# markomih/SplatFields

Hardware: AMD Instinct MI355X
Metric: splats*px rasterized/sec (fwd+bwd) (higher is better)
Workload: dtype f32

## Files before the change

splatfields_amd/csrc/api.hip:

```cpp
#include <cstdint>
#include <cstdio>
#include <cstdlib>
#include <cstring>
#include <atomic>
#include <chrono>
#include <thread>
#include <mutex>
#include <string>
#include <vector>
#include "host_api.h"
#include "kernels.h"

namespace {

thread_local std::string g_last_error;
thread_local long long g_last_longest = -1;

struct ProfRec { int stage; hipEvent_t a, b; bool ended; unsigned long long serial; };
unsigned long long g_prof_serial = 0;
bool g_prof_on = false;
std::vector<ProfRec> g_prof;
std::mutex g_prof_mutex;
const char* kStageNames[SR_PROFILE_STAGES] = {"preprocess", "scan", "emit", "sort_tiles", "render_forward",
                                              "render_backward", "preprocess_backward"};

}

namespace sr {

int fail(const std::string& msg) { g_last_error = msg; return 1; }

int check_hip(hipError_t e, const char* what) {
    if (e == hipSuccess) return 0;
    return fail(std::string(what) + ": " + hipGetErrorString(e));
}

StageTimer::StageTimer(int stage, hipStream_t s) : st(s) {
    if (!g_prof_on) return;
    ProfRec r; r.stage = stage; r.ended = false;
    if (hipEventCreate(&r.a) != hipSuccess || hipEventCreate(&r.b) != hipSuccess) return;
    hipEventRecord(r.a, st);
    std::lock_guard<std::mutex> lock(g_prof_mutex);
    serial = ++g_prof_serial;
    r.serial = serial;
    g_prof.push_back(r); idx = 0;
    end = r.b;
}
StageTimer::~StageTimer() {
    if (idx < 0) return;
    std::lock_guard<std::mutex> lock(g_prof_mutex);
    for (auto& r : g_prof)
        if (r.serial == serial) { hipEventRecord(end, st); r.ended = true; break; }
}

}

using sr::fail; using sr::check_hip; using sr::StageTimer;

namespace {

struct StatusBlock { uint32_t* pinned = nullptr; uint32_t* pinned_dev = nullptr; uint32_t seq = 0; hipStream_t stream = nullptr; int dev = 0; };
thread_local StatusBlock g_sync[64];
std::mutex g_ticket_mutex;
std::vector<StatusBlock*> g_ticket_free[64];
std::atomic<long long> g_counters[4];

int status_block_init(StatusBlock& b, int dev) {
    if (hipHostMalloc(reinterpret_cast<void**>(&b.pinned), 64, hipHostMallocCoherent) != hipSuccess &&
        hipHostMalloc(reinterpret_cast<void**>(&b.pinned), 64, hipHostMallocDefault) != hipSuccess) return fail("hipHostMalloc failed");
    void* dp = nullptr;
    if (hipHostGetDevicePointer(&dp, b.pinned, 0) != hipSuccess) { hipHostFree(b.pinned); b.pinned = nullptr; return fail("hipHostGetDevicePointer failed"); }
    b.pinned_dev = static_cast<uint32_t*>(dp);
    for (int i = 0; i < 16; ++i) b.pinned[i] = 0u;
    b.dev = dev; b.seq = 0;
    return 0;
}
uint32_t status_block_arm(StatusBlock& b, hipStream_t st) {
    b.seq = b.seq + 1u == 0u ? 1u : b.seq + 1u;
    b.stream = st;
    return b.seq;
}
int status_block_wait(StatusBlock& b, bool* waited) {
    volatile uint32_t* p = b.pinned;
    auto ready = [&] { return p[2] == b.seq && p[3] == b.seq; };
    if (waited) *waited = false;
    if (!ready()) {
        if (waited) *waited = true;
        const auto t0 = std::chrono::steady_clock::now();
        for (unsigned spins = 0; !ready(); ++spins) {
            if (spins > 4096u) std::this_thread::yield();
            if ((spins & 0xfffu) == 0xfffu && std::chrono::steady_clock::now() - t0 > std::chrono::seconds(2)) {
                SR_TRY(check_hip(hipStreamSynchronize(b.stream), "wait for the instance count"));
                if (!ready()) return fail("the instance count of the forward never reached the host (k_scan_small did not run?)");
            }
        }
    }
    std::atomic_thread_fence(std::memory_order_acquire);
    return 0;
}

int current_device(int* dev) {
    if (hipGetDevice(dev) != hipSuccess || *dev < 0 || *dev >= 64) return fail("hipGetDevice failed");
    return 0;
}

int thread_block(StatusBlock** out) {
    int dev = 0;
    SR_TRY(current_device(&dev));
    *out = &g_sync[dev];
    return (*out)->pinned ? 0 : status_block_init(**out, dev);
}

int ticket_acquire(StatusBlock** out) {
    int dev = 0;
    SR_TRY(current_device(&dev));
    {
        std::lock_guard<std::mutex> lock(g_ticket_mutex);
        if (!g_ticket_free[dev].empty()) { *out = g_ticket_free[dev].back(); g_ticket_free[dev].pop_back(); return 0; }
    }
    StatusBlock* t = new StatusBlock;
    if (int rc = status_block_init(*t, dev)) { delete t; return rc; }
    g_counters[3].fetch_add(1, std::memory_order_relaxed);
    *out = t;
    return 0;
}
void ticket_recycle(StatusBlock* t) {
    std::lock_guard<std::mutex> lock(g_ticket_mutex);
    g_ticket_free[t->dev].push_back(t);
}

std::atomic<int> g_bwd_kernel{[] {
    const char* sel = getenv("SPLATRASTER_BWD");
    return !sel ? 0 : (std::string(sel) == "wave" ? 1 : (std::string(sel) == "quads" ? 2 : 0));
}()};


struct CallContext { const SrView* view = nullptr; const SrSplats* splats = nullptr; const char* file = nullptr;
                     const float* dL_dcolor = nullptr; const float* dL_ddepth = nullptr; const float* dL_dalpha = nullptr; };
thread_local CallContext g_call;

void dump_record(FILE* f, const char* name, const void* dev, size_t bytes, bool on_device) {
    char tag[16] = {0};
    std::strncpy(tag, name, 15);
    std::vector<char> host;
    uint64_t n = 0;
    if (dev && bytes) {
        host.resize(bytes);
        if (!on_device) { std::memcpy(host.data(), dev, bytes); n = bytes; }
        else if (hipMemcpy(host.data(), dev, bytes, hipMemcpyDeviceToHost) == hipSuccess) n = bytes;
        else (void)hipGetLastError();
    }
    std::fwrite(tag, 1, 16, f); std::fwrite(&n, 8, 1, f);
    if (n) std::fwrite(host.data(), 1, (size_t)n, f);
}

void dump_snapshot(const char* stage) {
    const CallContext& c = g_call;
    if (!c.view || !c.splats || !c.file) return;
    FILE* f = std::fopen(c.file, "wb");
    if (!f) return;
    char head[8] = {'S', 'R', 'S', 'N', 'A', 'P', '1', 0}, st[32] = {0};
    std::strncpy(st, stage, 31);
    std::fwrite(head, 1, 8, f); std::fwrite(st, 1, 32, f);
    const SrView* v = c.view; const SrSplats* s = c.splats;
    const int32_t vi[4] = {v->image_height, v->image_width, v->sh_degree, v->sh_coeffs};
    const float vf[3] = {v->tanfovx, v->tanfovy, v->scale_modifier};
    char vb[32]; std::memcpy(vb, vi, 16); std::memcpy(vb + 16, vf, 12); const int32_t pf = v->prefiltered; std::memcpy(vb + 28, &pf, 4);
    dump_record(f, "view", vb, 32, false);
    const int32_t n = s->count;
    dump_record(f, "count", &n, 4, false);
    dump_record(f, "viewmatrix", v->viewmatrix, 64, true); dump_record(f, "projmatrix", v->projmatrix, 64, true);
    dump_record(f, "campos", v->campos, 12, true); dump_record(f, "bg", v->bg, 12, true);
    const size_t N = (size_t)(n > 0 ? n : 0);
    dump_record(f, "means3D", s->means3D, N * 12, true); dump_record(f, "opacities", s->opacities, N * 4, true);
    dump_record(f, "scales", s->scales, N * 12, true); dump_record(f, "rotations", s->rotations, N * 16, true);
    dump_record(f, "cov3D_precomp", s->cov3D_precomp, N * 24, true);
    dump_record(f, "shs", s->shs, s->shs ? N * 12 * (size_t)(s->shs_rest ? 1 : v->sh_coeffs) : 0, true);
    dump_record(f, "shs_rest", s->shs_rest, N * 12 * 15, true);
    dump_record(f, "colors_precomp", s->colors_precomp, N * 12, true);
    const size_t px = (size_t)v->image_height * v->image_width;
    dump_record(f, "dL_dcolor", c.dL_dcolor, px * 12, true); dump_record(f, "dL_ddepth", c.dL_ddepth, px * 4, true);
    dump_record(f, "dL_dalpha", c.dL_dalpha, px * 4, true);
    std::fclose(f);
}

int after_launch(const SrView* view, hipStream_t st, const char* what) {
    int rc = check_hip(hipGetLastError(), what);
    if (!rc && view && view->debug) rc = check_hip(hipStreamSynchronize(st), what);
    if (rc && view && view->debug) {
        const std::string keep = g_last_error;
        dump_snapshot(what);
        g_last_error = keep + (g_call.file ? std::string(" (inputs written to ") + g_call.file + ")" : std::string());
    }
    return rc;
}

int validate(const SrView* view, const SrSplats* s) {
    if (!view || !s) return fail("null view/splats");
    if (s->count < 0) return fail("negative splat count");
    if (view->image_height <= 0 || view->image_width <= 0) return fail("image size must be positive");
    if (!view->viewmatrix || !view->projmatrix || !view->campos || !view->bg) return fail("viewmatrix/projmatrix/campos/bg must be device pointers");
    if (s->count > 0) {
        if (!s->means3D || !s->opacities) return fail("means3D/opacities missing");
        const bool has_sr = s->scales && s->rotations;
        if (has_sr == (s->cov3D_precomp != nullptr)) return fail("Please provide exactly one of either scale/rotation pair or precomputed 3D covariance!");
        if ((s->shs != nullptr) == (s->colors_precomp != nullptr)) return fail("Please provide excatly one of either SHs or precomputed colors!");
        if (s->shs) {
            if (view->sh_degree < 0 || view->sh_degree > 3) return fail("sh_degree must be 0..3");
            if (view->sh_coeffs < (view->sh_degree + 1) * (view->sh_degree + 1)) return fail("shs holds fewer coefficients than sh_degree needs");
            if (s->shs_rest) {
                if (view->sh_coeffs != 16) return fail("shs_rest (dc + rest SH tensors) needs sh_coeffs == 16");
                if ((reinterpret_cast<uintptr_t>(s->shs) | reinterpret_cast<uintptr_t>(s->shs_rest)) & 15u) return fail("shs / shs_rest must be 16-byte aligned");
            }
        } else if (s->shs_rest) return fail("shs_rest without shs");
        if (s->raw_params & ~(SR_RAW_SCALES | SR_RAW_OPACITY | SR_RAW_ROTATIONS | SR_FORWARD_ONLY)) return fail("unknown bits in raw_params");
        if (s->cov3D_precomp && (s->raw_params & (SR_RAW_SCALES | SR_RAW_ROTATIONS))) return fail("raw scales/rotations with cov3D_precomp");
    }
    if ((sr::tiles_x(view->image_width) > sr::kMaxTilesPerSide) || (sr::tiles_y(view->image_height) > sr::kMaxTilesPerSide)) return fail("image too large (more than 65520 pixels a side)");
    return 0;
}

sr::ViewK make_view(const SrView* v) {
    sr::ViewK k;
    k.H = v->image_height; k.W = v->image_width;
    k.gx = sr::tiles_x(k.W); k.gy = sr::tiles_y(k.H);
    k.tanfovx = v->tanfovx; k.tanfovy = v->tanfovy;
    k.focal_x = k.W / (2.0f * v->tanfovx); k.focal_y = k.H / (2.0f * v->tanfovy);
    k.scale_modifier = v->scale_modifier;
    k.sh_degree = v->sh_degree; k.sh_coeffs = v->sh_coeffs;
    k.viewmatrix = v->viewmatrix; k.projmatrix = v->projmatrix; k.campos = v->campos; k.bg = v->bg;
    return k;
}

sr::SplatsK make_splats(const SrSplats* s) {
    sr::SplatsK k;
    k.N = s->count; k.means3D = s->means3D; k.opacities = s->opacities; k.scales = s->scales;
    k.rotations = s->rotations; k.cov3D = s->cov3D_precomp; k.shs = s->shs; k.colors = s->colors_precomp;
    k.raw = s->raw_params; k.shs_rest = s->shs_rest;
    return k;
}

long long covered_by_hint(long long hint) { return hint <= 2048 ? 2048 : hint <= 4096 ? 4096 : hint <= 8192 ? 8192 : -1; }

struct Call {
    hipStream_t st = nullptr;
    sr::ViewK v; sr::SplatsK s;
    sr::Geom g; sr::Binning b; sr::Image im;
    void carve(const void* geom, void* binning, long long capacity, const void* image) {
        sr::carve_geom(const_cast<void*>(geom), s.N, v.H, v.W, &g);
        if (binning) sr::carve_binning(binning, capacity, &b);
        if (image) sr::carve_image(const_cast<void*>(image), v.H, v.W, &im);
    }
};

int open_call(Call& c, const CallContext& ctx, void* hip_stream) {
    SR_TRY(validate(ctx.view, ctx.splats));
    g_call = ctx;
    c.st = static_cast<hipStream_t>(hip_stream);
    c.v = make_view(ctx.view);
    c.s = make_splats(ctx.splats);
    return 0;
}

bool capacity_in_range(long long r) { return r >= 0 && r < (1ll << 32); }

}

extern "C" {

int sr_version(void) { return SR_VERSION; }
const char* sr_last_error(void) { return g_last_error.c_str(); }

size_t sr_geom_bytes(int n, int h, int w) { return sr::carve_geom(nullptr, n, h, w, nullptr); }
size_t sr_binning_bytes(long long r, int, int) { return sr::carve_binning(nullptr, r, nullptr); }
size_t sr_image_bytes(int h, int w) { return sr::carve_image(nullptr, h, w, nullptr); }
size_t sr_backward_scratch_bytes(long long r) {
    const size_t n = (size_t)(r > 0 ? r : 1);
    return sr::align_up(n * sr::kSlotFloats * sizeof(float), 256);
}

}

namespace {

int launch_stage1(const SrView* view, const sr::ViewK& v, const sr::SplatsK& s, const sr::Geom& g, int* radii, uint32_t* host_out,
                  uint32_t host_seq, hipStream_t st) {
    { StageTimer t_(0, st); sr::launch_preprocess(v, s, g, radii, st); }
    SR_TRY(after_launch(view, st, "preprocess"));
    { StageTimer t_(1, st); sr::launch_count_tiles(v, s.N, g, st); sr::launch_scan_small(v, s.N, g, host_out, host_seq, st); }
    SR_TRY(after_launch(view, st, "scan"));
    return 0;
}

int launch_stage2(const SrView* view, const sr::ViewK& v, const sr::SplatsK& s, const sr::Geom& g, const sr::Binning& b,
                  const sr::Image& im, float* out_color, float* out_depth, float* out_alpha, StatusBlock* hs, long long max_len,
                  long long expected_len, hipStream_t st) {
    { StageTimer t_(2, st); sr::launch_emit(v, s.N, g, b, st); }
    SR_TRY(after_launch(view, st, "emit"));
    if (hs) {
        g_counters[0].fetch_add(1, std::memory_order_relaxed);
        SR_TRY(status_block_wait(*hs, nullptr));
        max_len = (long long)hs->pinned[1];
        if ((long long)hs->pinned[0] > (long long)b.capacity) return 0;
    }
    { StageTimer t_(3, st); sr::launch_sort_tiles(v, g, b, max_len, expected_len, st); }
    SR_TRY(after_launch(view, st, "sort_tiles"));
    { StageTimer t_(4, st); sr::launch_render_forward(v, g, b, im, out_color, out_depth, out_alpha, st); }
    SR_TRY(after_launch(view, st, "render_forward"));
    return 0;
}

}

extern "C" {

int sr_forward_prepare(const SrView* view, const SrSplats* splats, void* geom, int* radii,
                       long long* instances_out, void* hip_stream) {
    Call c;
    SR_TRY(open_call(c, CallContext{view, splats, "snapshot_fw.dump"}, hip_stream));
    if (!geom || !instances_out || (splats->count > 0 && !radii)) return fail("null geom/radii/instances_out");
    c.carve(geom, nullptr, 0, nullptr);
    StatusBlock* hs = nullptr;
    SR_TRY(thread_block(&hs));
    SR_TRY(launch_stage1(view, c.v, c.s, c.g, radii, hs->pinned_dev, status_block_arm(*hs, c.st), c.st));
    SR_TRY(check_hip(hipStreamSynchronize(c.st), "sync after prepare"));
    *instances_out = (long long)hs->pinned[0];
    return 0;
}

int sr_forward(const SrView* view, const SrSplats* splats, void* geom, int* radii, void* binning,
               long long binning_capacity, void* image, float* out_color, float* out_depth, float* out_alpha,
               long long* instances_out, void* hip_stream) {
    Call c;
    SR_TRY(open_call(c, CallContext{view, splats, "snapshot_fw.dump"}, hip_stream));
    if (!geom || !binning || !image || !out_color || !out_depth || !instances_out || (splats->count > 0 && !radii)) return fail("null buffer");
    if (!capacity_in_range(binning_capacity)) return fail("binning capacity out of range");
    c.carve(geom, binning, binning_capacity, image);
    StatusBlock* hs = nullptr;
    SR_TRY(thread_block(&hs));
    SR_TRY(launch_stage1(view, c.v, c.s, c.g, radii, hs->pinned_dev, status_block_arm(*hs, c.st), c.st));
    SR_TRY(launch_stage2(view, c.v, c.s, c.g, c.b, c.im, out_color, out_depth, out_alpha, hs, -1, -1, c.st));
    const long long total = (long long)hs->pinned[0];
    *instances_out = total;
    g_last_longest = (long long)hs->pinned[1];
    return total > binning_capacity ? SR_NEED_CAPACITY : 0;
}

int sr_forward_render(const SrView* view, const SrSplats* splats, void* geom, void* binning,
                      long long instances, void* image, float* out_color, float* out_depth,
                      float* out_alpha, void* hip_stream) {
    Call c;
    SR_TRY(open_call(c, CallContext{view, splats, "snapshot_fw.dump"}, hip_stream));
    if (!geom || !binning || !image || !out_color || !out_depth) return fail("null buffer");
    if (!capacity_in_range(instances)) return fail("instance count out of range");
    c.carve(geom, binning, instances, image);
    return launch_stage2(view, c.v, c.s, c.g, c.b, c.im, out_color, out_depth, out_alpha, nullptr, -1, -1, c.st);
}

int sr_forward_async(const SrView* view, const SrSplats* splats, void* geom, int* radii, void* binning,
                     long long binning_capacity, long long longest_list_hint, long long longest_list_expected, void* image,
                     float* out_color, float* out_depth, float* out_alpha, void** ticket_out, void* hip_stream) {
    Call c;
    SR_TRY(open_call(c, CallContext{view, splats, "snapshot_fw.dump"}, hip_stream));
    if (!geom || !binning || !image || !out_color || !out_depth || !ticket_out || (splats->count > 0 && !radii)) return fail("null buffer");
    if (!capacity_in_range(binning_capacity)) return fail("binning capacity out of range");
    if (longest_list_hint < 0) return fail("longest_list_hint must be >= 0");
    c.carve(geom, binning, binning_capacity, image);
    const long long covered = covered_by_hint(longest_list_hint);
    c.b.sorted_up_to = covered < 0 ? 0xffffffffu : (uint32_t)covered;
    StatusBlock* t = nullptr;
    SR_TRY(ticket_acquire(&t));
    int rc = launch_stage1(view, c.v, c.s, c.g, radii, t->pinned_dev, status_block_arm(*t, c.st), c.st);
    if (!rc) rc = launch_stage2(view, c.v, c.s, c.g, c.b, c.im, out_color, out_depth, out_alpha, nullptr, covered,
                                longest_list_expected >= 0 && longest_list_expected <= longest_list_hint ? longest_list_expected : -1, c.st);
    if (rc) {
        (void)hipStreamSynchronize(c.st);
        ticket_recycle(t);
        return rc;
    }
    g_counters[1].fetch_add(1, std::memory_order_relaxed);
    *ticket_out = t;
    return 0;
}

int sr_ticket_wait(void* ticket, long long* instances_out, long long* longest_list_out) {
    if (!ticket) return fail("null ticket");
    StatusBlock* t = static_cast<StatusBlock*>(ticket);
    bool waited = false;
    const int rc = status_block_wait(*t, &waited);
    if (waited) g_counters[2].fetch_add(1, std::memory_order_relaxed);
    if (rc) {
        return rc;
    }
    if (instances_out) *instances_out = (long long)t->pinned[0];
    if (longest_list_out) *longest_list_out = (long long)t->pinned[1];
    ticket_recycle(t);
    return 0;
}

long long sr_last_longest_list(void) { return g_last_longest; }

int sr_ticket_release(void* ticket) { return sr_ticket_wait(ticket, nullptr, nullptr); }

int sr_debug_counters(long long* out4, int reset) {
    if (!out4) return fail("null pointer in sr_debug_counters");
    for (int i = 0; i < 4; ++i) out4[i] = reset ? g_counters[i].exchange(0, std::memory_order_relaxed) : g_counters[i].load(std::memory_order_relaxed);
    return 0;
}

namespace {
int backward_impl(int what, const SrView* view, const SrSplats* splats, const void* geom, void* binning,
                  long long instances, long long instances_rendered, const void* image, const int* radii,
                  const float* dL_dcolor, const float* dL_ddepth, const float* dL_dalpha, void* scratch,
                  const SrGrads* grads, int first, int count, void* hip_stream) {
    Call c;
    SR_TRY(open_call(c, CallContext{view, splats, "snapshot_bw.dump", dL_dcolor, dL_ddepth, dL_dalpha}, hip_stream));
    if (!geom || !binning || !image || !scratch) return fail("null buffer");
    if ((what & 1) && !dL_dcolor) return fail("null buffer");
    if ((what & 2) && !grads) return fail("null buffer");
    if (what & 2) {
        if (splats->count > 0 && (!radii || !grads->dL_dmeans3D || !grads->dL_dmeans2D || !grads->dL_dopacity)) return fail("null gradient output");
        if (splats->count > 0 && splats->shs && !grads->dL_dshs && !grads->dL_dcolors) return fail("dL_dshs (or dL_dcolors for the colour-gradient mode) missing");
        if (splats->count > 0 && splats->shs_rest && grads->dL_dshs && !grads->dL_dshs_rest) return fail("dL_dshs_rest missing");
        if (splats->count > 0 && splats->colors_precomp && !grads->dL_dcolors) return fail("dL_dcolors missing");
        if (splats->count > 0 && splats->cov3D_precomp && !grads->dL_dcov3D) return fail("dL_dcov3D missing");
        if (splats->count > 0 && !splats->cov3D_precomp && (!grads->dL_dscales || !grads->dL_drotations)) return fail("dL_dscales/dL_drotations missing");
        if (first < 0 || count < 0 || (first % sr::kBlock) != 0) return fail("splat range must start at a multiple of 256");
    }
    if (splats->raw_params & SR_FORWARD_ONLY) return fail("the forward of these buffers was run with SR_FORWARD_ONLY");
    c.carve(geom, binning, instances, image);
    const hipStream_t st = c.st;
    const sr::SplatsK& s = c.s;
    float* slots = static_cast<float*>(scratch);
    if (what & 1) {
        StageTimer t_(5, st);
        const int pinned = g_bwd_kernel.load(std::memory_order_relaxed);
        const bool wave_kernel = pinned == 1;
        if (wave_kernel) sr::launch_render_backward(c.v, c.g, c.b, c.im, dL_dcolor, dL_ddepth, dL_dalpha, slots, st);
        else sr::launch_render_backward_quads(c.v, c.g, c.b, c.im, dL_dcolor, dL_ddepth, dL_dalpha, slots, st);
    }
    if (what & 1) SR_TRY(after_launch(view, st, "render_backward"));
    if (what & 2) {
        sr::GradsK gr;
        gr.means3D = grads->dL_dmeans3D; gr.means2D = grads->dL_dmeans2D; gr.opacity = grads->dL_dopacity;
        gr.scales = s.cov3D ? nullptr : grads->dL_dscales; gr.rotations = s.cov3D ? nullptr : grads->dL_drotations;
        gr.cov3D = s.cov3D ? grads->dL_dcov3D : nullptr;
        gr.shs = s.shs ? grads->dL_dshs : nullptr;
        gr.shs_rest = (s.shs_rest && gr.shs) ? grads->dL_dshs_rest : nullptr;
        gr.colors = (s.colors || (s.shs && !grads->dL_dshs)) ? grads->dL_dcolors : nullptr;
        const bool small_fp = !(instances_rendered >= 0 && instances_rendered > (long long)SR_BWD_SLOT_SPEC_BELOW * (long long)s.N);
        { StageTimer t_(6, st); sr::launch_preprocess_backward(c.v, s, c.g, radii, slots, c.b.reached, gr, first, count, small_fp, st); }
        SR_TRY(after_launch(view, st, "preprocess_backward"));
    }
    return 0;
}
}

int sr_backward(const SrView* view, const SrSplats* splats, const void* geom, void* binning,
                long long instances, long long instances_rendered, const void* image, const int* radii,
                const float* dL_dcolor, const float* dL_ddepth, const float* dL_dalpha, void* scratch,
                const SrGrads* grads, void* hip_stream) {
    return backward_impl(3, view, splats, geom, binning, instances, instances_rendered, image, radii, dL_dcolor, dL_ddepth, dL_dalpha,
                         scratch, grads, 0, splats ? splats->count : 0, hip_stream);
}

int sr_backward_blend(const SrView* view, const SrSplats* splats, const void* geom, void* binning,
                      long long instances, long long instances_rendered, const void* image,
                      const float* dL_dcolor, const float* dL_ddepth, const float* dL_dalpha, void* scratch, void* hip_stream) {
    return backward_impl(1, view, splats, geom, binning, instances, instances_rendered, image, nullptr, dL_dcolor, dL_ddepth, dL_dalpha,
                         scratch, nullptr, 0, 0, hip_stream);
}

int sr_backward_splats(const SrView* view, const SrSplats* splats, const void* geom, void* binning,
                       long long instances, long long instances_rendered, const void* image, const int* radii, void* scratch,
                       const SrGrads* grads, int first_splat, int n_splats, void* hip_stream) {
    return backward_impl(2, view, splats, geom, binning, instances, instances_rendered, image, radii, nullptr, nullptr, nullptr, scratch,
                         grads, first_splat, n_splats, hip_stream);
}

int sr_set_backward_kernel(int which) {
    if (which < 0 || which > 2) return -1;
    return g_bwd_kernel.exchange(which, std::memory_order_relaxed);
}

int sr_mark_visible(int n, const float* means3D, const float* viewmatrix, const float*, unsigned char* present, void* hip_stream) {
    if (n < 0 || (n > 0 && (!means3D || !viewmatrix || !present))) return fail("bad arguments to sr_mark_visible");
    hipStream_t st = static_cast<hipStream_t>(hip_stream);
    sr::launch_mark_visible(n, means3D, viewmatrix, present, st);
    return check_hip(hipGetLastError(), "mark_visible");
}

int sr_densification_stats(int n, const float* dL_dmeans2D, const int* radii, float* grad_accum, float* denom, float* max_radii2D,
                           void* hip_stream) {
    if (n < 0) return fail("bad arguments to sr_densification_stats");
    if (n > 0 && (!dL_dmeans2D || !radii)) return fail("null pointer in sr_densification_stats");
    sr::launch_densification_stats(n, dL_dmeans2D, radii, grad_accum, denom, max_radii2D, static_cast<hipStream_t>(hip_stream));
    return check_hip(hipGetLastError(), "densification_stats");
}

int sr_debug_layout(int n, int h, int w, long long instances, size_t* out4) {
    if (!out4 || n < 0 || h <= 0 || w <= 0 || instances < 0) return fail("bad arguments to sr_debug_layout");
    sr::Geom g; sr::Binning b;
    char* const origin = reinterpret_cast<char*>(4096);
    sr::carve_geom(origin, n, h, w, &g);
    sr::carve_binning(origin, instances, &b);
    out4[0] = (size_t)(reinterpret_cast<char*>(g.tile_start) - origin);
    out4[1] = (size_t)(reinterpret_cast<char*>(b.sorted_id) - origin);
    out4[2] = (size_t)(reinterpret_cast<char*>(g.total) - origin);
    out4[3] = (size_t)(reinterpret_cast<char*>(g.offsets) - origin);
    return 0;
}

int sr_debug_backward_stats(unsigned long long* out8, int reset) {
    if (!out8) return fail("null pointer in sr_debug_backward_stats");
    if (hipDeviceSynchronize() != hipSuccess) return fail("sr_debug_backward_stats: device synchronisation failed");
    return sr::backward_stats(out8, reset) ? fail("sr_debug_backward_stats: counter copy failed") : 0;
}

int sr_debug_snapshot(const SrView* view, const SrSplats* splats, const float* dL_dcolor, const float* dL_ddepth, const float* dL_dalpha,
                      int backward) {
    if (!view || !splats) return fail("null view/splats");
    g_call = CallContext{view, splats, backward ? "snapshot_bw.dump" : "snapshot_fw.dump", dL_dcolor, dL_ddepth, dL_dalpha};
    dump_snapshot(backward ? "render_backward (test hook)" : "preprocess (test hook)");
    return 0;
}

// ... 22 lines not shown
```

splatfields_amd/csrc/binning.hip:

```cpp
#include <atomic>
#include "kernels.h"
#include "expand.h"

namespace sr {

static void allow_dynamic_lds(const void* kernel, int slot, int bytes) {
    static std::atomic<bool> done[8][64];
    int dev = 0;
    if (hipGetDevice(&dev) != hipSuccess) return;
    if (dev >= 0 && dev < 64 && done[slot][dev].load(std::memory_order_acquire)) return;
    if (hipFuncSetAttribute(kernel, hipFuncAttributeMaxDynamicSharedMemorySize, bytes) != hipSuccess) { (void)hipGetLastError(); return; }
    if (dev >= 0 && dev < 64) done[slot][dev].store(true, std::memory_order_release);
}

__global__ void __launch_bounds__(kBlock) k_count_tiles(const ViewK v, int N, const Geom g, const Chunking ch) {
    extern __shared__ __attribute__((aligned(16))) uint32_t s_hist[];
    __shared__ uint32_t s_off[kBlock + 1];
    __shared__ ushort4 s_rect[kBlock];
    __shared__ float4 s_r0[kBlock], s_r1[kBlock];
    __shared__ uint32_t s_scan[8];
    for (int t = 4 * threadIdx.x; t < ch.tiles_padded; t += 4 * kBlock) *reinterpret_cast<uint4*>(&s_hist[t]) = make_uint4(0u, 0u, 0u, 0u);
    __syncthreads();
    const int base_chunk = (int)blockIdx.x / ch.slices, slice = (int)blockIdx.x % ch.slices;
    const int sb0 = base_chunk * ch.sub_per_chunk, sb1 = min(sb0 + ch.sub_per_chunk, ch.n_sub);
    for (int sb = sb0; sb < sb1; ++sb) {
        const int idx = sb * kBlock + threadIdx.x;
        uint32_t touched = 0;
        ushort4 rect = make_ushort4(0, 0, 0, 0);
        float4 r0 = make_float4(0.f, 0.f, -1.f, 0.f), r1 = r0;
        if (idx < N) {
            touched = g.touched[idx]; rect = g.rect[idx];
            if (touched > kMaskTiles) { r0 = g.rec[4 * (size_t)idx]; r1 = g.rec[4 * (size_t)idx + 1]; }
        }
        const uint32_t mask = rect_mask16(rect);
        const ushort4 packed = rect;
        rect = rect_clean(rect);
        const bool direct = ch.slices == 1 && touched <= kDirectTiles;
        if (direct && touched > 0u) {
            uint32_t k = 0;
            for (uint32_t ty = rect.y; ty < rect.w; ++ty)
                for (uint32_t tx = rect.x; tx < rect.z; ++tx, ++k)
                    if ((mask >> k) & 1u) atomicAdd(&s_hist[ty * (uint32_t)v.gx + tx], 1u);
        }
        const uint32_t coop = direct ? 0u : touched;
        if (!__syncthreads_or(coop != 0u)) continue;
        uint32_t total;
        const uint32_t excl = block_exclusive_scan(coop, s_scan, total);
        s_off[threadIdx.x] = excl;
        s_rect[threadIdx.x] = packed;
        tile_test_prepare(r0, r1, s_r0[threadIdx.x], s_r1[threadIdx.x]);
        if (threadIdx.x == 0) s_off[kBlock] = total;
        __syncthreads();
        for_each_block_instance(s_off, s_rect, v.gx, [&](int e, uint32_t k, uint32_t tile, uint32_t, uint32_t tile_x, uint32_t tile_y, uint32_t w) {
            if ((w & kRectMasked) ? (w >> k) & 1u : tile_reached(s_r0[e], s_r1[e], tile_x, tile_y)) atomicAdd(&s_hist[tile], 1u);
        }, (uint32_t)slice, (uint32_t)ch.slices);
    }
    __syncthreads();
    uint32_t* row = g.cnt + (size_t)blockIdx.x * ch.tiles_padded;
    for (int t = 4 * threadIdx.x; t < ch.tiles_padded; t += 4 * kBlock) *reinterpret_cast<uint4*>(&row[t]) = *reinterpret_cast<const uint4*>(&s_hist[t]);
}

#ifndef SR_STRIP_COLS
#define SR_STRIP_COLS 32
#endif
constexpr int kStripCols = SR_STRIP_COLS, kStripGroups = 1024 / kStripCols, kStripRows = (kMaxChunks + kStripGroups - 1) / kStripGroups;
__global__ void __launch_bounds__(1024) k_colscan(const Geom g, const Chunking ch) {
    __shared__ uint32_t s_tot[kStripGroups][kStripCols + 1];
    const int c = threadIdx.x % kStripCols, rg = threadIdx.x / kStripCols;
    const int col = blockIdx.x * kStripCols + c, row0 = rg * kStripRows;
    uint32_t* p = g.cnt + (size_t)row0 * ch.tiles_padded + col;
    uint32_t x[kStripRows];
#pragma unroll
    for (int r = 0; r < kStripRows; ++r) x[r] = row0 + r < ch.chunks ? p[(size_t)r * ch.tiles_padded] : 0u;
    uint32_t run = 0;
#pragma unroll
    for (int r = 0; r < kStripRows; ++r) { const uint32_t t = x[r]; x[r] = run; run += t; }
    s_tot[rg][c] = run;
    __syncthreads();
    uint32_t base = 0, all = 0;
#pragma unroll 8
    for (int k = 0; k < kStripGroups; ++k) { const uint32_t t = s_tot[k][c]; base += k < rg ? t : 0u; all += t; }
    if (rg == 0) g.segtot[col] = all;
#pragma unroll
    for (int r = 0; r < kStripRows; ++r) if (row0 + r < ch.chunks) p[(size_t)r * ch.tiles_padded] = x[r] + base;
}

void launch_count_tiles(const ViewK& v, int N, const Geom& g, hipStream_t st) {
    if (!use_count_matrix(v) || N <= 0) return;
    const Chunking ch = make_chunking(N, v.gx * v.gy);
    allow_dynamic_lds(reinterpret_cast<const void*>(&k_count_tiles), 0, (int)(sizeof(uint32_t) * kMaxMatrixTiles));
    hipLaunchKernelGGL(k_count_tiles, dim3(ch.chunks), dim3(kBlock), sizeof(uint32_t) * ch.tiles_padded, st, v, N, g, ch);
    hipLaunchKernelGGL(k_colscan, dim3(ch.tiles_padded / kStripCols), dim3(1024), 0, st, g, ch);
}

__global__ void __launch_bounds__(1024) k_scan_small(const Geom g, int n_sub, int n_tiles, const Chunking ch, int use_matrix,
                                                      uint32_t* __restrict__ host_out, uint32_t host_seq) {
    __shared__ uint32_t s_wave[16];
    const bool tiles = blockIdx.x == 1;
    uint32_t* dst = tiles ? g.tile_start : g.block_offsets;
    const int n = tiles ? n_tiles : n_sub;
    const int tid = threadIdx.x, lane = tid & 63, w = tid >> 6;
    constexpr int kPer = 4;
    uint32_t carry = 0, vmax = 0;
    uint32_t v[kPer];
    for (int base = 0; base < n; base += 1024 * kPer) {
        const int i0 = base + tid * kPer;
        uint32_t sum = 0;
#pragma unroll
        for (int k = 0; k < kPer; ++k) {
            const int i = i0 + k;
            v[k] = 0;
            if (i < n) {
                if (!tiles) v[k] = g.block_sums[i];
                else if (!use_matrix) v[k] = g.tile_count[i];
                else v[k] = g.segtot[i];
            }
            vmax = max(vmax, v[k]);
            sum += v[k];
        }
        const uint32_t inc = wave_inclusive_scan(sum);
        if (lane == 63) s_wave[w] = inc;
        __syncthreads();
        uint32_t wave_base = 0, all = 0;
#pragma unroll
        for (int k = 0; k < 16; ++k) { const uint32_t t = s_wave[k]; if (k < w) wave_base += t; all += t; }
        uint32_t run = carry + wave_base + inc - sum;
#pragma unroll
        for (int k = 0; k < kPer; ++k) {
            const int i = i0 + k;
            if (i < n) { dst[i] = run; if (tiles) g.tile_cursor[i] = 0u; }
            run += v[k];
        }
        carry += all;
        __syncthreads();
    }
    const bool in_regs = n <= 1024 * kPer;
    if (tid == 0) {
        if (tiles) dst[n] = carry;
        else {
            g.total[0] = carry;
            if (host_out) { host_out[0] = carry; __hip_atomic_store(host_out + 2, host_seq, __ATOMIC_RELEASE, __HIP_MEMORY_SCOPE_SYSTEM); }
        }
    }
    if (tiles) {
#pragma unroll
        for (int d = 32; d > 0; d >>= 1) vmax = max(vmax, (uint32_t)__shfl_xor((int)vmax, d, 64));
        __syncthreads();
        if (lane == 0) s_wave[w] = vmax;
        __syncthreads();
        if (tid == 0) {
            uint32_t m = 0;
            for (int k = 0; k < 16; ++k) m = max(m, s_wave[k]);
            g.total[1] = m; s_wave[0] = m;
            if (host_out) { host_out[1] = m; __hip_atomic_store(host_out + 3, host_seq, __ATOMIC_RELEASE, __HIP_MEMORY_SCOPE_SYSTEM); }
        }
        __syncthreads();
        __shared__ uint32_t s_hist[256];
        const uint32_t longest = max(s_wave[0], 1u);
        const float to_class = 255.0f / (float)longest;
        if (tid < 256) s_hist[tid] = 0u;
        __syncthreads();
        if (in_regs) {
#pragma unroll
            for (int k = 0; k < kPer; ++k)
                if (tid * kPer + k < n) atomicAdd(&s_hist[255u - min(255u, (uint32_t)((float)v[k] * to_class))], 1u);
        } else {
            for (int i = tid; i < n; i += 1024) {
                const uint32_t len = dst[i + 1] - dst[i];
                atomicAdd(&s_hist[255u - min(255u, (uint32_t)((float)len * to_class))], 1u);
            }
        }
        __syncthreads();
        if (w == 0) {
            uint32_t c0 = s_hist[4 * lane], c1 = s_hist[4 * lane + 1], c2 = s_hist[4 * lane + 2], c3 = s_hist[4 * lane + 3];
            const uint32_t sum = c0 + c1 + c2 + c3;
            const uint32_t excl = wave_inclusive_scan(sum) - sum;
            s_hist[4 * lane] = excl; s_hist[4 * lane + 1] = excl + c0; s_hist[4 * lane + 2] = excl + c0 + c1;
            s_hist[4 * lane + 3] = excl + c0 + c1 + c2;
        }
        __syncthreads();
        if (tid < 3) {
            const uint32_t lo = 2048u << tid;
            uint32_t cand = 0u;
            if (longest > lo) {
                const uint32_t cls = 255u - min(255u, (uint32_t)((float)(lo + 1u) * to_class));
                cand = cls >= 255u ? (uint32_t)n : s_hist[cls + 1u];
            }
            g.total[4 + tid] = cand;
        }
        __syncthreads();
        if (in_regs) {
#pragma unroll
            for (int k = 0; k < kPer; ++k)
                if (tid * kPer + k < n)
                    g.tile_order[atomicAdd(&s_hist[255u - min(255u, (uint32_t)((float)v[k] * to_class))], 1u)] = (uint32_t)(tid * kPer + k);
        } else {
            for (int i = tid; i < n; i += 1024) {
                const uint32_t len = dst[i + 1] - dst[i];
                g.tile_order[atomicAdd(&s_hist[255u - min(255u, (uint32_t)((float)len * to_class))], 1u)] = (uint32_t)i;
            }
        }
    }
}

void launch_scan_small(const ViewK& v, int N, const Geom& g, uint32_t* host_out, uint32_t host_seq, hipStream_t st) {
    const Chunking ch = make_chunking(N, v.gx * v.gy);
    hipLaunchKernelGGL(k_scan_small, dim3(2), dim3(1024), 0, st, g, (N + kBlock - 1) / kBlock, v.gx * v.gy, ch,
                       use_count_matrix(v) ? 1 : 0, host_out, host_seq);
}

template <bool MATRIX>
__global__ void __launch_bounds__(kBlock) k_emit(const ViewK v, int N, const Geom g, const Binning b, const Chunking ch) {
    extern __shared__ __attribute__((aligned(16))) uint32_t s_cur[];
    __shared__ uint32_t s_off[kBlock + 1];
    __shared__ ushort4 s_rect[kBlock];
    __shared__ uint32_t s_depth[kBlock];
    __shared__ float4 s_r0[kBlock], s_r1[kBlock];
    __shared__ uint32_t s_scan[8];
    if (g.total[0] > b.capacity) return;
    int sb0 = blockIdx.x, sb1 = blockIdx.x + 1;
    uint32_t slice = 0, slices = 1;
    if constexpr (MATRIX) {
        const int per = (ch.chunks + 7) >> 3;
        const int chunk = (int)(blockIdx.x & 7u) * per + (int)(blockIdx.x >> 3);
        if ((int)(blockIdx.x >> 3) >= per || chunk >= ch.chunks) return;
        slice = (uint32_t)(chunk % ch.slices); slices = (uint32_t)ch.slices;
        sb0 = (chunk / ch.slices) * ch.sub_per_chunk; sb1 = min(sb0 + ch.sub_per_chunk, ch.n_sub);
        const uint32_t* row = g.cnt + (size_t)chunk * ch.tiles_padded;
        const int n_tiles = v.gx * v.gy;
        for (int t = 4 * threadIdx.x; t < n_tiles; t += 4 * kBlock) {
            const uint4 a = *reinterpret_cast<const uint4*>(&g.tile_start[t]), r = *reinterpret_cast<const uint4*>(&row[t]);
            *reinterpret_cast<uint4*>(&s_cur[t]) = make_uint4(a.x + r.x, a.y + r.y, a.z + r.z, a.w + r.w);
        }
    }
    constexpr int kAhead = 4;
    for (int sbg = sb0; sbg < sb1; sbg += kAhead) {
        uint32_t touched_a[kAhead], word_a[kAhead], dbits_a[kAhead], base_a[kAhead];
        ushort4 rect_a[kAhead];
        float4 r0_a[kAhead], r1_a[kAhead];
#pragma unroll
        for (int u = 0; u < kAhead; ++u) {
            const int idx = (sbg + u) * kBlock + threadIdx.x;
            touched_a[u] = 0; dbits_a[u] = 0; base_a[u] = 0; rect_a[u] = make_ushort4(0, 0, 0, 0);
            if (sbg + u < sb1) {
                base_a[u] = g.block_offsets[sbg + u];
                if (idx < N) {
                    touched_a[u] = g.touched[idx];
                    rect_a[u] = g.rect[idx];
                    dbits_a[u] = g.depth_bits[idx];
                }
            }
        }
#pragma unroll
        for (int u = 0; u < kAhead; ++u) {
            const int idx = (sbg + u) * kBlock + threadIdx.x;
            r0_a[u] = make_float4(0.f, 0.f, -1.f, 0.f); r1_a[u] = r0_a[u];
            if (touched_a[u] > kMaskTiles) { r0_a[u] = g.rec[4 * (size_t)idx]; r1_a[u] = g.rec[4 * (size_t)idx + 1]; }
            word_a[u] = rect_mask16(rect_a[u]);
        }
#pragma unroll
        for (int u = 0; u < kAhead; ++u) {
            const int sb = sbg + u;
            if (sb >= sb1) break;
            const int idx = sb * kBlock + threadIdx.x;
            const uint32_t touched = touched_a[u], mask = word_a[u];
            const bool direct = slices == 1u && touched <= kDirectTiles;
            const uint32_t coop = direct ? 0u : touched;
            uint32_t total, coop_total;
            uint32_t coop_excl;
            const uint32_t excl = block_exclusive_scan2(touched, coop, s_scan, total, coop_excl, coop_total);
            const uint32_t base = base_a[u];
            if (idx < N) g.offsets[idx] = base + excl;
            if (slice == 0u)
                for (uint32_t i = threadIdx.x; i < total; i += kBlock) b.reached[base + i] = 0;
            const uint32_t first_splat = (uint32_t)sb * kBlock;
            if (direct && touched > 0u) {
                const uint64_t entry = ((uint64_t)dbits_a[u] << 32) | (uint64_t)(first_splat + threadIdx.x);
                uint32_t k = 0;
                const ushort4 rc = rect_clean(rect_a[u]);
                for (uint32_t ty = rc.y; ty < rc.w; ++ty)
                    for (uint32_t tx = rc.x; tx < rc.z; ++tx, ++k) {
                        if (!((mask >> k) & 1u)) continue;
                        const uint32_t tile = ty * (uint32_t)v.gx + tx;
                        uint32_t slot;
                        if constexpr (MATRIX) slot = atomicAdd(&s_cur[tile], 1u);
                        else slot = g.tile_start[tile] + atomicAdd(&g.tile_cursor[tile], 1u);
                        b.ent[slot] = entry;
                    }
            }
            if (coop_total == 0u) continue;
            s_off[threadIdx.x] = coop_excl;
            s_rect[threadIdx.x] = rect_a[u];
            s_depth[threadIdx.x] = dbits_a[u];
            tile_test_prepare(r0_a[u], r1_a[u], s_r0[threadIdx.x], s_r1[threadIdx.x]);
            if (threadIdx.x == 0) s_off[kBlock] = coop_total;
            __syncthreads();
            for_each_block_instance(s_off, s_rect, v.gx, [&](int e, uint32_t k, uint32_t tile, uint32_t, uint32_t tile_x, uint32_t tile_y, uint32_t w) {
                if (!((w & kRectMasked) ? (w >> k) & 1u : tile_reached(s_r0[e], s_r1[e], tile_x, tile_y))) return;
                uint32_t slot;
                if constexpr (MATRIX) slot = atomicAdd(&s_cur[tile], 1u);
                else slot = g.tile_start[tile] + atomicAdd(&g.tile_cursor[tile], 1u);
                b.ent[slot] = ((uint64_t)s_depth[e] << 32) | (uint64_t)(first_splat + (uint32_t)e);
            }, slice, slices);
        }
    }
}

void launch_emit(const ViewK& v, int N, const Geom& g, const Binning& b, hipStream_t st) {
    if (N <= 0) return;
    const Chunking ch = make_chunking(N, v.gx * v.gy);
    allow_dynamic_lds(reinterpret_cast<const void*>(&k_emit<true>), 1, (int)(sizeof(uint32_t) * kMaxMatrixTiles));
    if (use_count_matrix(v))
        hipLaunchKernelGGL(k_emit<true>, dim3((ch.chunks + 7) / 8 * 8), dim3(kBlock), sizeof(uint32_t) * ch.tiles_padded, st, v, N, g, b, ch);
    else
        hipLaunchKernelGGL(k_emit<false>, dim3(ch.n_sub), dim3(kBlock), 0, st, v, N, g, b, ch);
}

template <int D>
__device__ __forceinline__ uint32_t lane_xor(uint32_t x) {
    if constexpr (D == 1) return (uint32_t)__builtin_amdgcn_update_dpp(0, (int)x, 0xB1, 0xf, 0xf, false);
    else if constexpr (D == 2) return (uint32_t)__builtin_amdgcn_update_dpp(0, (int)x, 0x4E, 0xf, 0xf, false);
    else if constexpr (D == 8) return (uint32_t)__builtin_amdgcn_update_dpp(0, (int)x, 0x128, 0xf, 0xf, false);
    else if constexpr (D == 4) {
        const uint32_t a = (uint32_t)__builtin_amdgcn_update_dpp(0, (int)x, 0x124, 0xf, 0xf, false);
        const uint32_t b = (uint32_t)__builtin_amdgcn_update_dpp(0, (int)x, 0x12C, 0xf, 0xf, false);
        return (threadIdx.x & 4u) ? a : b;
    } else if constexpr (D == 16) {
        typedef unsigned int u2 __attribute__((ext_vector_type(2)));
        const u2 r = __builtin_amdgcn_permlane16_swap(x, x, false, false);
        return (threadIdx.x & 16u) ? r.x : r.y;
    } else {
        typedef unsigned int u2 __attribute__((ext_vector_type(2)));
        const u2 r = __builtin_amdgcn_permlane32_swap(x, x, false, false);
        return (threadIdx.x & 32u) ? r.x : r.y;
    }
}

__device__ __forceinline__ uint32_t lane_xor_d(uint32_t x, int d) {
    switch (d) {
        case 1: return lane_xor<1>(x);
        case 2: return lane_xor<2>(x);
        case 4: return lane_xor<4>(x);
        case 8: return lane_xor<8>(x);
        case 16: return lane_xor<16>(x);
        default: return lane_xor<32>(x);
    }
}

__device__ __forceinline__ void exchange_select(uint64_t& k, uint64_t pk, bool keep_min) {
    const bool take = (pk < k) == keep_min;
    k = take ? pk : k;
}

template <int N, int E>
__device__ __forceinline__ void bitonic_regs(uint64_t (&k)[E], uint64_t* skey, uint32_t tid) {
#pragma unroll
    for (int kk = 2; kk <= N; kk <<= 1) {
#pragma unroll
        for (int j = kk >> 1; j > 0; j >>= 1) {
            if (j < E) {
#pragma unroll
                for (int e = 0; e < E; ++e) {
                    if ((e & j) == 0) {
                        const uint32_t i = tid * E + e;
                        const bool asc = (i & kk) == 0;
                        const bool swap = (k[e] > k[e | j]) == asc;
                        const uint64_t ka = k[e], kb = k[e | j];
                        k[e] = swap ? kb : ka; k[e | j] = swap ? ka : kb;
                    }
                }
            } else if (j < 64 * E) {
                const int d = j / E;
                const bool lower = (tid & d) == 0;
                const bool keep_min = lower == (((tid * E) & kk) == 0);
                uint32_t plo[E], phi[E];
#pragma unroll
                for (int e = 0; e < E; ++e) {
                    plo[e] = lane_xor_d((uint32_t)k[e], d);
                    phi[e] = lane_xor_d((uint32_t)(k[e] >> 32), d);
                }
#pragma unroll
                for (int e = 0; e < E; ++e) exchange_select(k[e], ((uint64_t)phi[e] << 32) | plo[e], keep_min);
            } else {
                __syncthreads();
#pragma unroll
                for (int e = 0; e < E; ++e) skey[tid * E + e] = k[e];
                __syncthreads();
#pragma unroll
                for (int e = 0; e < E; ++e) {
                    const uint32_t i = tid * E + e;
                    const bool asc = (i & kk) == 0;
                    const bool lower = (i & j) == 0;
                    exchange_select(k[e], skey[i ^ j], lower == asc);
                }
            }
        }
    }
}

template <int N, int E>
__device__ __forceinline__ void load_sort_chunk(const Binning& b, uint32_t first, uint32_t m, uint64_t (&k)[E], uint64_t* scratch_key, uint32_t tid) {
#pragma unroll
    for (int e = 0; e < E; ++e) {
        const uint32_t i = tid * E + e;
        k[e] = i < m ? b.ent[first + i] : ~0ull;
    }
    bitonic_regs<N, E>(k, scratch_key, tid);
}

template <int N, int E>
__device__ __forceinline__ void sort_tile_regs(const Binning& b, uint32_t start, uint32_t n, uint64_t* skey) {
    uint64_t k[E];
    load_sort_chunk<N, E>(b, start, n, k, skey, threadIdx.x);
#pragma unroll
    for (int e = 0; e < E; ++e) {
        const uint32_t i = threadIdx.x * E + e;
        if (i < n) b.sorted_id[start + i] = (uint32_t)k[e];
    }
}

template <int CAP, int THREADS, typename Emit>
__device__ __forceinline__ void sort_block_lds(const Binning& b, uint32_t first, uint32_t n, uint64_t* run_key, Emit&& emit);

__global__ void __launch_bounds__(256) k_sort_tiles_regs(const Geom g, const Binning b) {
    __shared__ uint64_t skey[2048];
    const uint32_t total_instances = g.total[0];
    const uint32_t tile = g.tile_order[blockIdx.x];
    asm volatile("" :: "s"(tile));
    if (total_instances > b.capacity) return;
    const uint32_t start = g.tile_start[tile];
    const uint32_t n = g.tile_start[tile + 1] - start;
    if (n == 0u || n > 2048u) return;
    if (n <= 256u) sort_tile_regs<256, 1>(b, start, n, skey);
    else if (n <= 512u) sort_tile_regs<512, 2>(b, start, n, skey);
    else if (n <= 1024u) sort_tile_regs<1024, 4>(b, start, n, skey);
    else sort_block_lds<2048, 256>(b, start, n, skey, [&](uint32_t rank, uint64_t key) { b.sorted_id[start + rank] = (uint32_t)key; });
}

template <int E, typename Out>
__device__ __forceinline__ void merge_run_pairs(const uint64_t* src, uint32_t n, uint32_t width, Out&& out) {
    const uint32_t o = threadIdx.x * (uint32_t)E;
    if (o >= n) return;
    const uint32_t base = o & ~(2u * width - 1u);
    const uint64_t* A = src + base;
    const uint32_t a = min(width, n - base);
    const uint32_t b = n - base - a < width ? n - base - a : width;
    const uint32_t d = o - base;
    uint32_t lo = d > b ? d - b : 0u, hi = min(d, a);
    while (lo < hi) {
        const uint32_t mid = (lo + hi) >> 1;
        if (A[mid] < A[width + d - 1u - mid]) lo = mid + 1u; else hi = mid;
    }
    uint32_t ai = lo, bi = d - lo;
    constexpr uint64_t kInf = ~0ull;
    uint64_t ka = ai < a ? A[ai] : kInf;
    uint64_t kb = bi < b ? A[width + bi] : kInf;
#pragma unroll
    for (int e = 0; e < E; ++e) {
        const bool take_a = ka < kb;
        const uint64_t key = take_a ? ka : kb;
        if (d + (uint32_t)e < a + b) out(o + (uint32_t)e, key);
        ai += take_a ? 1u : 0u;
        bi += take_a ? 0u : 1u;
        const bool more = take_a ? ai < a : bi < b;
        const uint64_t nxt = A[take_a ? min(ai, a - 1u) : width + min(bi, max(b, 1u) - 1u)];
        if (take_a) ka = more ? nxt : kInf; else kb = more ? nxt : kInf;
    }
}
// ... 127 lines not shown
```

splatfields_amd/csrc/kernels.h:

```cpp
#pragma once
#include "common.h"

namespace sr {

struct SplatsK {
    int N;
    const float* means3D; const float* opacities; const float* scales; const float* rotations;
    const float* cov3D; const float* shs; const float* colors;
    int raw;
    const float* shs_rest;
};

struct GradsK {
    float* means3D; float* means2D; float* opacity; float* scales; float* rotations; float* cov3D;
    float* shs; float* colors; float* shs_rest;
};

void launch_preprocess(const ViewK& v, const SplatsK& s, const Geom& g, int* radii, hipStream_t st);
void launch_mark_visible(int N, const float* means3D, const float* viewmatrix, unsigned char* present, hipStream_t st);
void launch_densification_stats(int N, const float* dL_dmeans2D, const int* radii, float* grad_accum, float* denom, float* max_radii2D,
                                hipStream_t st);
void launch_preprocess_backward(const ViewK& v, const SplatsK& s, const Geom& g, const int* radii,
                                const float* slots, const uint8_t* reached, const GradsK& gr, int first, int count, bool small_footprint,
                                hipStream_t st);
inline bool use_count_matrix(const ViewK& v) { return v.gx * v.gy <= kMaxMatrixTiles; }
void launch_count_tiles(const ViewK& v, int N, const Geom& g, hipStream_t st);
void launch_scan_small(const ViewK& v, int N, const Geom& g, uint32_t* host_out, uint32_t host_seq, hipStream_t st);
void launch_emit(const ViewK& v, int N, const Geom& g, const Binning& b, hipStream_t st);
void launch_sort_tiles(const ViewK& v, const Geom& g, const Binning& b, long long max_len, long long expected_len, hipStream_t st);
void launch_render_forward(const ViewK& v, const Geom& g, const Binning& b, const Image& im,
                           float* out_color, float* out_depth, float* out_alpha, hipStream_t st);
void launch_render_backward(const ViewK& v, const Geom& g, const Binning& b, const Image& im,
                            const float* dL_dcolor, const float* dL_ddepth, const float* dL_dalpha,
                            float* slots, hipStream_t st);
void launch_render_backward_quads(const ViewK& v, const Geom& g, const Binning& b, const Image& im,
                                 const float* dL_dcolor, const float* dL_ddepth, const float* dL_dalpha,
                                 float* slots, hipStream_t st);

int backward_stats(unsigned long long* out8, int reset);

}
```

Baseline: 1317000 billion.

## Fold small prefix-scan kernel into column-scan and emit kernels

Removes the separate k_scan_small launch when the count matrix path is used. The sub-block offset scan moves into an extra last block of k_colscan, and the tile-start scan into an extra first block of k_emit. Each emit block now recomputes its tile base offsets from the per-tile totals with a block-wide scan. This saves one kernel launch and its serialization, at the cost of redundant per-block scan work in emit and a more complex host-status handoff.

```diff
diff --git a/splatfields_amd/csrc/api.hip b/splatfields_amd/csrc/api.hip
--- a/splatfields_amd/csrc/api.hip
+++ b/splatfields_amd/csrc/api.hip
@@ -91,7 +91,7 @@
             if (spins > 4096u) std::this_thread::yield();
             if ((spins & 0xfffu) == 0xfffu && std::chrono::steady_clock::now() - t0 > std::chrono::seconds(2)) {
                 SR_TRY(check_hip(hipStreamSynchronize(b.stream), "wait for the instance count"));
-                if (!ready()) return fail("the instance count of the forward never reached the host (k_scan_small did not run?)");
+                if (!ready()) return fail("the instance count of the forward never reached the host (did the small prefix sums not run?)");
             }
         }
     }
@@ -287,15 +287,19 @@
                   uint32_t host_seq, hipStream_t st) {
     { StageTimer t_(0, st); sr::launch_preprocess(v, s, g, radii, st); }
     SR_TRY(after_launch(view, st, "preprocess"));
-    { StageTimer t_(1, st); sr::launch_count_tiles(v, s.N, g, st); sr::launch_scan_small(v, s.N, g, host_out, host_seq, st); }
+    {
+        StageTimer t_(1, st);
+        sr::launch_count_tiles(v, s.N, g, host_out, host_seq, st);
+        if (!sr::scan_is_folded(v, s.N)) sr::launch_scan_small(v, s.N, g, host_out, host_seq, st);
+    }
     SR_TRY(after_launch(view, st, "scan"));
     return 0;
 }
 
 int launch_stage2(const SrView* view, const sr::ViewK& v, const sr::SplatsK& s, const sr::Geom& g, const sr::Binning& b,
-                  const sr::Image& im, float* out_color, float* out_depth, float* out_alpha, StatusBlock* hs, long long max_len,
-                  long long expected_len, hipStream_t st) {
-    { StageTimer t_(2, st); sr::launch_emit(v, s.N, g, b, st); }
+                  const sr::Image& im, float* out_color, float* out_depth, float* out_alpha, StatusBlock* pub, StatusBlock* hs,
+                  long long max_len, long long expected_len, hipStream_t st) {
+    { StageTimer t_(2, st); sr::launch_emit(v, s.N, g, b, pub ? pub->pinned_dev : nullptr, pub ? pub->seq : 0u, st); }
     SR_TRY(after_launch(view, st, "emit"));
     if (hs) {
         g_counters[0].fetch_add(1, std::memory_order_relaxed);
@@ -339,7 +343,7 @@
     StatusBlock* hs = nullptr;
     SR_TRY(thread_block(&hs));
     SR_TRY(launch_stage1(view, c.v, c.s, c.g, radii, hs->pinned_dev, status_block_arm(*hs, c.st), c.st));
-    SR_TRY(launch_stage2(view, c.v, c.s, c.g, c.b, c.im, out_color, out_depth, out_alpha, hs, -1, -1, c.st));
+    SR_TRY(launch_stage2(view, c.v, c.s, c.g, c.b, c.im, out_color, out_depth, out_alpha, hs, hs, -1, -1, c.st));
     const long long total = (long long)hs->pinned[0];
     *instances_out = total;
     g_last_longest = (long long)hs->pinned[1];
@@ -354,7 +358,7 @@
     if (!geom || !binning || !image || !out_color || !out_depth) return fail("null buffer");
     if (!capacity_in_range(instances)) return fail("instance count out of range");
     c.carve(geom, binning, instances, image);
-    return launch_stage2(view, c.v, c.s, c.g, c.b, c.im, out_color, out_depth, out_alpha, nullptr, -1, -1, c.st);
+    return launch_stage2(view, c.v, c.s, c.g, c.b, c.im, out_color, out_depth, out_alpha, nullptr, nullptr, -1, -1, c.st);
 }
 
 int sr_forward_async(const SrView* view, const SrSplats* splats, void* geom, int* radii, void* binning,
@@ -371,7 +375,7 @@
     StatusBlock* t = nullptr;
     SR_TRY(ticket_acquire(&t));
     int rc = launch_stage1(view, c.v, c.s, c.g, radii, t->pinned_dev, status_block_arm(*t, c.st), c.st);
-    if (!rc) rc = launch_stage2(view, c.v, c.s, c.g, c.b, c.im, out_color, out_depth, out_alpha, nullptr, covered,
+    if (!rc) rc = launch_stage2(view, c.v, c.s, c.g, c.b, c.im, out_color, out_depth, out_alpha, t, nullptr, covered,
                                 longest_list_expected >= 0 && longest_list_expected <= longest_list_hint ? longest_list_expected : -1, c.st);
     if (rc) {
         (void)hipStreamSynchronize(c.st);
diff --git a/splatfields_amd/csrc/binning.hip b/splatfields_amd/csrc/binning.hip
--- a/splatfields_amd/csrc/binning.hip
+++ b/splatfields_amd/csrc/binning.hip
@@ -63,9 +63,17 @@
 #ifndef SR_STRIP_COLS
 #define SR_STRIP_COLS 32
 #endif
+template <int THREADS>
+__device__ __forceinline__ void scan_small_half(const Geom& g, int n_sub, int n_tiles, int use_matrix, uint32_t* __restrict__ host_out,
+                                                uint32_t host_seq, bool tiles);
+
 constexpr int kStripCols = SR_STRIP_COLS, kStripGroups = 1024 / kStripCols, kStripRows = (kMaxChunks + kStripGroups - 1) / kStripGroups;
-__global__ void __launch_bounds__(1024) k_colscan(const Geom g, const Chunking ch) {
+__global__ void __launch_bounds__(1024) k_colscan(const Geom g, const Chunking ch, uint32_t* __restrict__ host_out, uint32_t host_seq) {
     __shared__ uint32_t s_tot[kStripGroups][kStripCols + 1];
+    if (blockIdx.x == gridDim.x - 1) {
+        scan_small_half<1024>(g, ch.n_sub, 0, 1, host_out, host_seq, false);
+        return;
+    }
     const int c = threadIdx.x % kStripCols, rg = threadIdx.x / kStripCols;
     const int col = blockIdx.x * kStripCols + c, row0 = rg * kStripRows;
     uint32_t* p = g.cnt + (size_t)row0 * ch.tiles_padded + col;
@@ -85,25 +93,26 @@
     for (int r = 0; r < kStripRows; ++r) if (row0 + r < ch.chunks) p[(size_t)r * ch.tiles_padded] = x[r] + base;
 }
 
-void launch_count_tiles(const ViewK& v, int N, const Geom& g, hipStream_t st) {
-    if (!use_count_matrix(v) || N <= 0) return;
+void launch_count_tiles(const ViewK& v, int N, const Geom& g, uint32_t* host_out, uint32_t host_seq, hipStream_t st) {
+    if (!scan_is_folded(v, N)) return;
     const Chunking ch = make_chunking(N, v.gx * v.gy);
     allow_dynamic_lds(reinterpret_cast<const void*>(&k_count_tiles), 0, (int)(sizeof(uint32_t) * kMaxMatrixTiles));
     hipLaunchKernelGGL(k_count_tiles, dim3(ch.chunks), dim3(kBlock), sizeof(uint32_t) * ch.tiles_padded, st, v, N, g, ch);
-    hipLaunchKernelGGL(k_colscan, dim3(ch.tiles_padded / kStripCols), dim3(1024), 0, st, g, ch);
-}
-
-__global__ void __launch_bounds__(1024) k_scan_small(const Geom g, int n_sub, int n_tiles, const Chunking ch, int use_matrix,
-                                                      uint32_t* __restrict__ host_out, uint32_t host_seq) {
+    hipLaunchKernelGGL(k_colscan, dim3(ch.tiles_padded / kStripCols + 1), dim3(1024), 0, st, g, ch, host_out, host_seq);
+}
+
+template <int THREADS>
+__device__ __forceinline__ void scan_small_half(const Geom& g, int n_sub, int n_tiles, int use_matrix, uint32_t* __restrict__ host_out,
+                                                uint32_t host_seq, bool tiles) {
+    constexpr int kWaves = THREADS / 64;
     __shared__ uint32_t s_wave[16];
-    const bool tiles = blockIdx.x == 1;
     uint32_t* dst = tiles ? g.tile_start : g.block_offsets;
     const int n = tiles ? n_tiles : n_sub;
     const int tid = threadIdx.x, lane = tid & 63, w = tid >> 6;
-    constexpr int kPer = 4;
+    constexpr int kPer = 4096 / THREADS;
     uint32_t carry = 0, vmax = 0;
     uint32_t v[kPer];
-    for (int base = 0; base < n; base += 1024 * kPer) {
+    for (int base = 0; base < n; base += THREADS * kPer) {
         const int i0 = base + tid * kPer;
         uint32_t sum = 0;
 #pragma unroll
@@ -123,7 +132,7 @@
         __syncthreads();
         uint32_t wave_base = 0, all = 0;
 #pragma unroll
-        for (int k = 0; k < 16; ++k) { const uint32_t t = s_wave[k]; if (k < w) wave_base += t; all += t; }
+        for (int k = 0; k < kWaves; ++k) { const uint32_t t = s_wave[k]; if (k < w) wave_base += t; all += t; }
         uint32_t run = carry + wave_base + inc - sum;
 #pragma unroll
         for (int k = 0; k < kPer; ++k) {
@@ -134,7 +143,7 @@
         carry += all;
         __syncthreads();
     }
-    const bool in_regs = n <= 1024 * kPer;
+    const bool in_regs = n <= THREADS * kPer;
     if (tid == 0) {
         if (tiles) dst[n] = carry;
         else {
@@ -150,7 +159,7 @@
         __syncthreads();
         if (tid == 0) {
             uint32_t m = 0;
-            for (int k = 0; k < 16; ++k) m = max(m, s_wave[k]);
+            for (int k = 0; k < kWaves; ++k) m = max(m, s_wave[k]);
             g.total[1] = m; s_wave[0] = m;
             if (host_out) { host_out[1] = m; __hip_atomic_store(host_out + 3, host_seq, __ATOMIC_RELEASE, __HIP_MEMORY_SCOPE_SYSTEM); }
         }
@@ -165,7 +174,7 @@
             for (int k = 0; k < kPer; ++k)
                 if (tid * kPer + k < n) atomicAdd(&s_hist[255u - min(255u, (uint32_t)((float)v[k] * to_class))], 1u);
         } else {
-            for (int i = tid; i < n; i += 1024) {
+            for (int i = tid; i < n; i += THREADS) {
                 const uint32_t len = dst[i + 1] - dst[i];
                 atomicAdd(&s_hist[255u - min(255u, (uint32_t)((float)len * to_class))], 1u);
             }
@@ -195,12 +204,17 @@
                 if (tid * kPer + k < n)
                     g.tile_order[atomicAdd(&s_hist[255u - min(255u, (uint32_t)((float)v[k] * to_class))], 1u)] = (uint32_t)(tid * kPer + k);
         } else {
-            for (int i = tid; i < n; i += 1024) {
+            for (int i = tid; i < n; i += THREADS) {
                 const uint32_t len = dst[i + 1] - dst[i];
                 g.tile_order[atomicAdd(&s_hist[255u - min(255u, (uint32_t)((float)len * to_class))], 1u)] = (uint32_t)i;
             }
         }
     }
+}
+
+__global__ void __launch_bounds__(1024) k_scan_small(const Geom g, int n_sub, int n_tiles, const Chunking ch, int use_matrix,
+                                                      uint32_t* __restrict__ host_out, uint32_t host_seq) {
+    scan_small_half<1024>(g, n_sub, n_tiles, use_matrix, host_out, host_seq, blockIdx.x == 1);
 }
 
 void launch_scan_small(const ViewK& v, int N, const Geom& g, uint32_t* host_out, uint32_t host_seq, hipStream_t st) {
@@ -210,27 +224,45 @@
 }
 
 template <bool MATRIX>
-__global__ void __launch_bounds__(kBlock) k_emit(const ViewK v, int N, const Geom g, const Binning b, const Chunking ch) {
+__global__ void __launch_bounds__(kBlock) k_emit(const ViewK v, int N, const Geom g, const Binning b, const Chunking ch,
+                                                  uint32_t* __restrict__ host_out, uint32_t host_seq) {
     extern __shared__ __attribute__((aligned(16))) uint32_t s_cur[];
     __shared__ uint32_t s_off[kBlock + 1];
     __shared__ ushort4 s_rect[kBlock];
     __shared__ uint32_t s_depth[kBlock];
     __shared__ float4 s_r0[kBlock], s_r1[kBlock];
     __shared__ uint32_t s_scan[8];
+    if constexpr (MATRIX) {
+        if (blockIdx.x == 0u) {
+            scan_small_half<kBlock>(g, 0, v.gx * v.gy, 1, host_out, host_seq, true);
+            return;
+        }
+    }
     if (g.total[0] > b.capacity) return;
-    int sb0 = blockIdx.x, sb1 = blockIdx.x + 1;
+    const uint32_t bid = MATRIX ? blockIdx.x - 1u : blockIdx.x;
+    int sb0 = bid, sb1 = bid + 1;
     uint32_t slice = 0, slices = 1;
     if constexpr (MATRIX) {
         const int per = (ch.chunks + 7) >> 3;
-        const int chunk = (int)(blockIdx.x & 7u) * per + (int)(blockIdx.x >> 3);
-        if ((int)(blockIdx.x >> 3) >= per || chunk >= ch.chunks) return;
+        const int chunk = (int)(bid & 7u) * per + (int)(bid >> 3);
+        if ((int)(bid >> 3) >= per || chunk >= ch.chunks) return;
         slice = (uint32_t)(chunk % ch.slices); slices = (uint32_t)ch.slices;
         sb0 = (chunk / ch.slices) * ch.sub_per_chunk; sb1 = min(sb0 + ch.sub_per_chunk, ch.n_sub);
         const uint32_t* row = g.cnt + (size_t)chunk * ch.tiles_padded;
-        const int n_tiles = v.gx * v.gy;
-        for (int t = 4 * threadIdx.x; t < n_tiles; t += 4 * kBlock) {
-            const uint4 a = *reinterpret_cast<const uint4*>(&g.tile_start[t]), r = *reinterpret_cast<const uint4*>(&row[t]);
-            *reinterpret_cast<uint4*>(&s_cur[t]) = make_uint4(a.x + r.x, a.y + r.y, a.z + r.z, a.w + r.w);
+        const int per_t = ((ch.tiles_padded + kBlock - 1) / kBlock + 3) & ~3;
+        const int t0 = min((int)threadIdx.x * per_t, ch.tiles_padded), t1 = min(t0 + per_t, ch.tiles_padded);
+        uint32_t sum = 0;
+        for (int t = t0; t < t1; t += 4) {
+            const uint4 a = *reinterpret_cast<const uint4*>(&g.segtot[t]);
+            *reinterpret_cast<uint4*>(&s_cur[t]) = a;
+            sum += a.x + a.y + a.z + a.w;
+        }
+        uint32_t all;
+        uint32_t run = block_exclusive_scan(sum, s_scan, all);
+        for (int t = t0; t < t1; t += 4) {
+            const uint4 a = *reinterpret_cast<const uint4*>(&s_cur[t]), r = *reinterpret_cast<const uint4*>(&row[t]);
+            *reinterpret_cast<uint4*>(&s_cur[t]) = make_uint4(run + r.x, run + a.x + r.y, run + a.x + a.y + r.z, run + a.x + a.y + a.z + r.w);
+            run += a.x + a.y + a.z + a.w;
         }
     }
     constexpr int kAhead = 4;
@@ -306,14 +338,15 @@
     }
 }
 
-void launch_emit(const ViewK& v, int N, const Geom& g, const Binning& b, hipStream_t st) {
+void launch_emit(const ViewK& v, int N, const Geom& g, const Binning& b, uint32_t* host_out, uint32_t host_seq, hipStream_t st) {
     if (N <= 0) return;
     const Chunking ch = make_chunking(N, v.gx * v.gy);
     allow_dynamic_lds(reinterpret_cast<const void*>(&k_emit<true>), 1, (int)(sizeof(uint32_t) * kMaxMatrixTiles));
     if (use_count_matrix(v))
-        hipLaunchKernelGGL(k_emit<true>, dim3((ch.chunks + 7) / 8 * 8), dim3(kBlock), sizeof(uint32_t) * ch.tiles_padded, st, v, N, g, b, ch);
+        hipLaunchKernelGGL(k_emit<true>, dim3((ch.chunks + 7) / 8 * 8 + 1), dim3(kBlock), sizeof(uint32_t) * ch.tiles_padded, st, v, N, g, b, ch,
+                           host_out, host_seq);
     else
-        hipLaunchKernelGGL(k_emit<false>, dim3(ch.n_sub), dim3(kBlock), 0, st, v, N, g, b, ch);
+        hipLaunchKernelGGL(k_emit<false>, dim3(ch.n_sub), dim3(kBlock), 0, st, v, N, g, b, ch, nullptr, 0u);
 }
 
 template <int D>
diff --git a/splatfields_amd/csrc/kernels.h b/splatfields_amd/csrc/kernels.h
--- a/splatfields_amd/csrc/kernels.h
+++ b/splatfields_amd/csrc/kernels.h
@@ -24,9 +24,10 @@
                                 const float* slots, const uint8_t* reached, const GradsK& gr, int first, int count, bool small_footprint,
                                 hipStream_t st);
 inline bool use_count_matrix(const ViewK& v) { return v.gx * v.gy <= kMaxMatrixTiles; }
-void launch_count_tiles(const ViewK& v, int N, const Geom& g, hipStream_t st);
+inline bool scan_is_folded(const ViewK& v, int N) { return use_count_matrix(v) && N > 0; }
+void launch_count_tiles(const ViewK& v, int N, const Geom& g, uint32_t* host_out, uint32_t host_seq, hipStream_t st);
 void launch_scan_small(const ViewK& v, int N, const Geom& g, uint32_t* host_out, uint32_t host_seq, hipStream_t st);
-void launch_emit(const ViewK& v, int N, const Geom& g, const Binning& b, hipStream_t st);
+void launch_emit(const ViewK& v, int N, const Geom& g, const Binning& b, uint32_t* host_out, uint32_t host_seq, hipStream_t st);
 void launch_sort_tiles(const ViewK& v, const Geom& g, const Binning& b, long long max_len, long long expected_len, hipStream_t st);
 void launch_render_forward(const ViewK& v, const Geom& g, const Binning& b, const Image& im,
                            float* out_color, float* out_depth, float* out_alpha, hipStream_t st);
```

Result: faster. 1330000 billion (median of 4 runs) (+1.0%).
